# podmortem/log-parser

Hardware: AMD Instinct MI355X
Metric: log-lines/sec parsed+scored (whole node), 1k-pattern library (higher is better)
Workload: dtype fp64

## Files before the change

### csrc/bind.cpp

```cpp
#include <pybind11/numpy.h>
#include <pybind11/pybind11.h>
#include <pybind11/stl.h>

#include <atomic>
#include <chrono>
#include <condition_variable>
#include <cstring>
#include <deque>
#include <memory>
#include <mutex>
#include <thread>

#include "io/docs.h"
#include "io/json_in.h"
#include "io/loadgen.h"
#include "io/http_server.h"
#include "io/json_emit.h"
#include "kernels/lp_api.h"
#include "kernels/lp_host.h"
#include "regex/jregex.h"
#include "runtime/proc_shared.h"
#include "runtime/request.h"

namespace py = pybind11;
using namespace lp;

template <typename T>
static T* P(uint64_t v) { return reinterpret_cast<T*>(v); }

static PfTables pf_from(const py::tuple& t) {
  PfTables T;
  T.bloom = P<const uint32_t>(t[0].cast<uint64_t>());
  T.bloom_bits = t[1].cast<int>();
  T.ht_key = P<const uint64_t>(t[2].cast<uint64_t>());
  T.ht_val = P<const int32_t>(t[3].cast<uint64_t>());
  T.ht_cnt = P<const int32_t>(t[4].cast<uint64_t>());
  T.ht_mask = t[5].cast<uint32_t>();
  T.gram_lits = P<const int32_t>(t[6].cast<uint64_t>());
  T.lit_off = P<const int32_t>(t[7].cast<uint64_t>());
  T.lit_bytes = P<const uint8_t>(t[8].cast<uint64_t>());
  T.lit_reg_off = P<const int32_t>(t[9].cast<uint64_t>());
  T.lit_reg = P<const int32_t>(t[10].cast<uint64_t>());
  T.gmask = t[11].cast<int>();
  T.stride = t[12].cast<int>();
  T.teddy = P<const uint32_t>(t[13].cast<uint64_t>());
  T.tb_off = P<const int32_t>(t[14].cast<uint64_t>());
  T.tb_lits = P<const int32_t>(t[15].cast<uint64_t>());
  T.teddy_on = t[16].cast<int>();
  if (t.size() > 18) {
    T.gram_fp = P<const uint64_t>(t[17].cast<uint64_t>());
    T.tb_fp = P<const uint64_t>(t[18].cast<uint64_t>());
  }
  return T;
}

static DfaPool dfa_from(const py::tuple& t) {
  DfaPool D;
  D.meta = P<const int32_t>(t[0].cast<uint64_t>());
  D.bytemap = P<const uint8_t>(t[1].cast<uint64_t>());
  D.trans = P<const uint16_t>(t[2].cast<uint64_t>());
  D.acc = P<const uint8_t>(t[3].cast<uint64_t>());
  D.bpg = t.size() > 4 ? P<const uint64_t>(t[4].cast<uint64_t>()) : nullptr;
  D.bpg_widths = t.size() > 5 ? t[5].cast<uint32_t>() : 0u;
  D.bpg_words = t.size() > 6 ? t[6].cast<uint32_t>() : 0u;
  return D;
}

static GapTab gt_from(const py::tuple& t) {
  GapTab T;
  T.key = P<int64_t>(t[0].cast<uint64_t>());
  T.count = P<unsigned long long>(t[1].cast<uint64_t>());
  T.first = P<long long>(t[2].cast<uint64_t>());
  T.docs = P<int32_t>(t[3].cast<uint64_t>());
  T.last_doc = P<int32_t>(t[4].cast<uint64_t>());
  T.used = P<unsigned long long>(t[5].cast<uint64_t>());
  T.cap = t[6].cast<int64_t>();
  return T;
}

static GapRows gr_from(const py::tuple& t) {
  GapRows R;
  R.sig = P<int64_t>(t[0].cast<uint64_t>());
  R.count = P<int64_t>(t[1].cast<uint64_t>());
  R.first = P<int64_t>(t[2].cast<uint64_t>());
// ... 805 lines not shown
    return py::make_tuple(py::bytes(out.data(), k), intact);
  });

  m.def("line_index_tiles", &line_index_tiles);
  m.def("line_index_dev", [](uint64_t text, int64_t n, uint64_t ws, int64_t ntiles_cap, uint64_t starts, uint64_t lens,
                             int64_t cap, uint64_t info, bool trim, uint64_t blk, int64_t nblk, uint64_t s, bool counted) {
    line_index_dev(P<const uint8_t>(text), n, LineIndexWs{P<int64_t>(ws), ntiles_cap, size_t(1) << 20}, P<int64_t>(starts),
                   P<int32_t>(lens), cap, P<int64_t>(info), trim, P<int32_t>(blk), nblk, s, counted); },
        py::arg("text"), py::arg("n"), py::arg("ws"), py::arg("ntiles_cap"), py::arg("starts"), py::arg("lens"),
        py::arg("cap"), py::arg("info"), py::arg("trim"), py::arg("blk"), py::arg("nblk"), py::arg("s"),
        py::arg("counted") = false);
  m.def("prefilter_dev", [](uint64_t text, int64_t n, py::tuple pf, uint64_t ls, int64_t nl, uint64_t cand, int64_t cap,
                            uint64_t count, int grid, uint64_t s, py::object nlp) {
    NlOut o;
    const bool fused = !nlp.is_none();
    if (fused) {
      py::tuple t = nlp.cast<py::tuple>();
      o.nlm = P<uint64_t>(t[0].cast<uint64_t>());
      o.cnt = P<int32_t>(t[1].cast<uint64_t>());
      o.crf = P<int32_t>(t[2].cast<uint64_t>());
      o.ntiles = t[3].cast<int64_t>();
    }
    prefilter_dev(P<const uint8_t>(text), n, pf_from(pf), P<const int64_t>(ls), nl, P<int64_t>(cand), cap,
                  P<unsigned long long>(count), grid, s, fused ? &o : nullptr); },
        py::arg("text"), py::arg("n"), py::arg("pf"), py::arg("ls"), py::arg("nl"), py::arg("cand"), py::arg("cap"),
        py::arg("count"), py::arg("grid"), py::arg("s"), py::arg("nlp") = py::none());
  m.def("line_index_pass1", [](uint64_t ws, int64_t ntiles_cap, int64_t n, uint64_t s) {
    const NlOut o = line_index_pass1_views(LineIndexWs{P<int64_t>(ws), ntiles_cap, size_t(1) << 20}, n, s);
    return py::make_tuple(reinterpret_cast<uint64_t>(o.nlm), reinterpret_cast<uint64_t>(o.cnt),
                          reinterpret_cast<uint64_t>(o.crf), o.ntiles);
  });
  m.def("pf_verify_dev", [](uint64_t gh, int64_t n, uint64_t text, int64_t nb, py::tuple pf, uint64_t ls, int64_t nl,
                            uint64_t blk, uint64_t cand, int64_t cap, uint64_t count, uint64_t s, uint64_t dn,
                            int max_grid) {
    pf_verify_dev(P<const int64_t>(gh), n, P<const uint8_t>(text), nb, pf_from(pf), P<const int64_t>(ls), nl,
                  P<const int32_t>(blk), P<int64_t>(cand), cap, P<unsigned long long>(count), s,
                  P<const unsigned long long>(dn), max_grid); }, py::arg("gh"), py::arg("n"), py::arg("text"),
        py::arg("nb"), py::arg("pf"), py::arg("ls"), py::arg("nl"), py::arg("blk"), py::arg("cand"), py::arg("cap"),
        py::arg("count"), py::arg("s"), py::arg("dn") = 0, py::arg("max_grid") = 8192);
  m.def("append_keys", [](uint64_t dst, int64_t cap, uint64_t count, uint64_t src, int64_t n, uint64_t s) {
    append_keys_dev(P<int64_t>(dst), cap, P<unsigned long long>(count), P<const int64_t>(src), n, s); });
  m.def("take_host", [](uint64_t cand, uint64_t n1d, int64_t cap1, uint64_t ver, uint64_t n2d, int64_t cap2,
                        uint64_t text, uint64_t ls, uint64_t ll, py::tuple dfa, py::object out, uint64_t s) {
    HostSideOut O;
    if (!out.is_none()) {
      py::tuple t = out.cast<py::tuple>();
      O.keys = P<int64_t>(t[0].cast<uint64_t>()); O.starts = P<int64_t>(t[1].cast<uint64_t>());
      O.lens = P<int64_t>(t[2].cast<uint64_t>()); O.cap = t[3].cast<int64_t>();
      O.cnt = P<unsigned long long>(t[4].cast<uint64_t>()); O.done_blocks = P<unsigned int>(t[5].cast<uint64_t>());
      O.host_cnt = P<int64_t>(t[6].cast<uint64_t>()); O.host_seq = P<int64_t>(t[7].cast<uint64_t>());
      O.seq = t[8].cast<int64_t>();
    }
    take_host_dev(P<int64_t>(cand), P<const unsigned long long>(n1d), cap1, P<int64_t>(ver),
                  P<const unsigned long long>(n2d), cap2, P<const uint8_t>(text), P<const int64_t>(ls),
                  P<const int32_t>(ll), dfa_from(dfa), O, s); });
  m.def("wait_host", [](uint64_t ver, int64_t cap2, uint64_t n2d, py::tuple in, uint64_t s, double timeout_s) {
    HostSideIn I;
    I.keys = P<const int64_t>(in[0].cast<uint64_t>()); I.host_cnt = P<const int64_t>(in[1].cast<uint64_t>());
    I.host_seq = P<const int64_t>(in[2].cast<uint64_t>()); I.cap = in[3].cast<int64_t>(); I.seq = in[4].cast<int64_t>();
    I.err = P<int64_t>(in[5].cast<uint64_t>());
    I.timeout_ticks = (long long)(timeout_s * 1e8);
    wait_host_dev(P<int64_t>(ver), cap2, P<unsigned long long>(n2d), I, s); }, py::arg("ver"), py::arg("cap2"),
    py::arg("n2d"), py::arg("in"), py::arg("stream"), py::arg("timeout_s") = 2.0);
  m.def("host_alloc_coherent", [](int64_t bytes) {
    void* h = nullptr;
    if (hipHostMalloc(&h, (size_t)std::max<int64_t>(bytes, 8), hipHostMallocMapped | hipHostMallocCoherent) != hipSuccess)
      throw std::runtime_error("hipHostMalloc (coherent) failed");
    std::memset(h, 0, (size_t)std::max<int64_t>(bytes, 8));
    void* d = nullptr;
    if (hipHostGetDevicePointer(&d, h, 0) != hipSuccess) {
      (void)hipHostFree(h);
      throw std::runtime_error("hipHostGetDevicePointer failed");
// ... 697 lines not shown
```

### csrc/kernels/lp_api.h

```cpp
#pragma once
#include <stdint.h>

#include <vector>

#include "lp_core.h"

namespace lp {

void set_host_threads(int n);
void set_pf_verify_lanes(int n);
bool scan_defer_rare();
void set_scan_defer_rare(bool on);
void set_cand_verify_split(bool on);
bool summ_select();
void set_summ_select(bool on);
void set_small_profile(uint64_t dev_ptr);
struct NlOut {
  uint64_t* nlm = nullptr;
  int32_t* cnt = nullptr;
  int32_t* crf = nullptr;
  int64_t ntiles = 0;
};
void prefilter_dev(const uint8_t* text, int64_t nbytes, const PfTables& T, const int64_t* line_start, int64_t nlines,
                   int64_t* cand, int64_t cap, unsigned long long* count, int grid, uint64_t stream,
                   const NlOut* nl = nullptr);
void pf_verify_dev(const int64_t* ghits, int64_t n, const uint8_t* text, int64_t nbytes, const PfTables& T,
                   const int64_t* line_start, int64_t nlines, const int32_t* blk_line, int64_t* cand, int64_t cap,
                   unsigned long long* count, uint64_t stream, const unsigned long long* dn = nullptr,
                   int max_grid = 8192);
void bpg_cand_dev(int64_t* cand, int64_t cap, const unsigned long long* dcount, const uint8_t* text, const int64_t* ls,
                  const int32_t* ll, const DfaPool& P, uint64_t stream);
bool cand_verify_all_dev(int64_t* cand, int64_t cap, const unsigned long long* dcount, const uint8_t* text,
                         const int64_t* ls, const int32_t* ll, const DfaPool& P, uint64_t stream);
bool bpg_dedupe_dev(const uint64_t* keys, int64_t n, int lbits, const uint8_t* text, const int64_t* ls,
                    const int32_t* ll, const DfaPool& P, uint8_t* flag, uint64_t stream, uint32_t* wcnt = nullptr,
                    uint32_t* wlist = nullptr, int64_t* std_key = nullptr);
void bpg_scan_dev(const uint8_t* text, const int64_t* ls, const int32_t* ll, int64_t L, const int32_t* regs,
                  int nregs, const DfaPool& P, int64_t* out, int64_t cap, unsigned long long* count,
                  uint64_t stream);
struct HostSideOut {
  int64_t* keys = nullptr;
  int64_t* starts = nullptr;
  int64_t* lens = nullptr;
  int64_t cap = 0;
  unsigned long long* cnt = nullptr;
  unsigned int* done_blocks = nullptr;
  int64_t* host_cnt = nullptr;
  int64_t* host_seq = nullptr;
  int64_t seq = 0;
};
struct HostSideIn {
  const int64_t* keys = nullptr;
  const int64_t* host_cnt = nullptr;
  const int64_t* host_seq = nullptr;
  int64_t cap = 0;
  int64_t seq = 0;
  long long timeout_ticks = 200000000;
  int64_t* err = nullptr;
};
void take_host_dev(int64_t* cand, const unsigned long long* n1d, int64_t cap1, int64_t* ver,
                   const unsigned long long* n2d, int64_t cap2, const uint8_t* text, const int64_t* ls,
                   const int32_t* ll, const DfaPool& P, const HostSideOut& O, uint64_t stream);
// ... 334 lines not shown
```

### csrc/kernels/lp_core.h

```cpp
#pragma once
#include <hip/hip_runtime.h>
#include <stdint.h>

#define LP_HD __host__ __device__ __forceinline__

namespace lp {

template <typename T, int U = 8>
__device__ __forceinline__ void lds_fill(T* dst, const T* __restrict__ src, int n) {
  for (int b = threadIdx.x; b < n; b += U * (int)blockDim.x) {
    T v[U];
#pragma unroll
    for (int j = 0; j < U; ++j) {
      const int i = b + j * (int)blockDim.x;
      v[j] = src[i < n ? i : n - 1];
    }
#pragma unroll
    for (int j = 0; j < U; ++j) {
      const int i = b + j * (int)blockDim.x;
      if (i < n) dst[i] = v[j];
    }
  }
}

// ... 131 lines not shown
  if (ftl) {
    for (int k = 0; k < 4; ++k)
      if (st[k] >= 2 && (D[k].A[st[k]] & 2)) st[k] = 1;
    advance(s + ft, ftl);
  }
  uint32_t res = 0;
  for (int k = 0; k < 4; ++k)
    if (st[k] == 1 || (st[k] >= 2 && (D[k].A[st[k]] & 1))) res |= 1u << k;
  const uint8_t f = (res & 1u) ? 1 : ((res & 2u) ? 2 : 0);
  return (uint8_t)(f | (res & 12u));
#endif
}

struct PfTables {
  const uint32_t* bloom;
  int bloom_bits;
  const uint64_t* ht_key;
  const int32_t* ht_val;
  const int32_t* ht_cnt;
  uint32_t ht_mask;
  const int32_t* gram_lits;
  const int32_t* lit_off;
  const uint8_t* lit_bytes;
  const int32_t* lit_reg_off;
  const int32_t* lit_reg;
  int gmask;
  int stride;
  const uint32_t* teddy;
  const int32_t* tb_off;
  const int32_t* tb_lits;
  int teddy_on;
  const uint64_t* gram_fp = nullptr;
  const uint64_t* tb_fp = nullptr;
};

constexpr int LIT_OFF_SHIFT = 22;
LP_HD int pf_entry_lit(int32_t e) { return e & ((1 << LIT_OFF_SHIFT) - 1); }
LP_HD int pf_entry_off(int32_t e) { return (int)((uint32_t)e >> LIT_OFF_SHIFT); }

LP_HD uint32_t gram_mask(int g) { return g >= 4 ? 0xFFFFFFFFu : ((1u << (8 * g)) - 1u); }
LP_HD uint32_t bloom_hash(uint32_t key, int g) { return (key ^ (uint32_t)g * 0x9E3779B9u) * 0x85EBCA6Bu; }
LP_HD uint32_t bloom_word(uint32_t key, int g, int bits) {
  return bloom_hash(key, g) >> (32 - (bits - 5));
}
LP_HD uint32_t bloom_bits_of(uint32_t p) {
  const uint32_t q = p ^ (p >> 15);
  return (1u << (q & 31)) | (1u << ((q >> 5) & 31)) | (1u << ((q >> 10) & 31));
}
LP_HD uint32_t bloom_bits2(uint32_t key, int g) { return bloom_bits_of(bloom_hash(key, g)); }
LP_HD bool bloom_test(const uint32_t* bl, uint32_t key, int g, int bits) {
  const uint32_t p = bloom_hash(key, g);
  const uint32_t m = bloom_bits_of(p);
  return (bl[p >> (32 - (bits - 5))] & m) == m;
}
LP_HD uint32_t ht_hash(uint32_t key, int g) {
  uint32_t h = key * 0x9E3779B1u ^ ((uint32_t)g * 0x7FEB352Du);
  h ^= h >> 15;
  h *= 0x2C1B3C6Du;
  h ^= h >> 12;
  return h;
}
LP_HD int lower_byte(int c) { return (c >= 'A' && c <= 'Z') ? c + 32 : c; }
LP_HD uint32_t lower4(uint32_t x) {
  uint32_t hi = 0x80808080u;
  uint32_t ge_A = ((x | hi) - 0x41414141u) & hi;
  uint32_t ge_Z1 = ((x | hi) - 0x5B5B5B5Bu) & hi;
  uint32_t up = ge_A & ~ge_Z1 & ~x & hi;
// ... 33 lines not shown
#if defined(__HIP__)
__device__ __forceinline__ void load16u(const uint8_t* p, uint32_t out[4]) {
  const int sh = (int)((uintptr_t)p & 15);
  const uint4* b = reinterpret_cast<const uint4*>(p - sh);
  const uint4 x = b[0], y = b[1];
  uint32_t a0 = x.x, a1 = x.y, a2 = x.z, a3 = x.w, a4 = y.x, a5 = y.y, a6 = y.z, a7 = y.w;
  const int q = sh >> 2, r = sh & 3;
  if (q & 2) { a0 = a2; a1 = a3; a2 = a4; a3 = a5; a4 = a6; a5 = a7; }
  if (q & 1) { a0 = a1; a1 = a2; a2 = a3; a3 = a4; a4 = a5; }
  out[0] = __builtin_amdgcn_alignbyte(a1, a0, r);
  out[1] = __builtin_amdgcn_alignbyte(a2, a1, r);
  out[2] = __builtin_amdgcn_alignbyte(a3, a2, r);
  out[3] = __builtin_amdgcn_alignbyte(a4, a3, r);
}
__device__ __forceinline__ bool lit_match16(const uint8_t* t, const uint8_t* lit, int len) {
  for (int q = 0; q < len; q += 16) {
    uint32_t a[4], b[4];
    load16u(t + q, a);
    load16u(lit + q, b);
    const int rem = len - q;
    uint32_t diff = 0;
#pragma unroll
    for (int i = 0; i < 4; ++i) {
      const int k = rem - 4 * i;
      const uint32_t m = k >= 4 ? 0xFFFFFFFFu : (k <= 0 ? 0u : ((1u << (8 * k)) - 1u));
      diff |= (lower4(a[i]) ^ b[i]) & m;
    }
    if (diff) return false;
  }
  return true;
}
#endif

LP_HD void pf_bucket(const PfTables& T, uint32_t gram, int g, int& s, int& c) {
  const uint64_t key = (uint64_t)gram | ((uint64_t)g << 32);
  uint32_t h = ht_hash(gram, g) & T.ht_mask;
  s = 0;
  c = 0;
  for (;;) {
    const uint64_t kk = T.ht_key[h];
    if (kk == ~0ull) return;
    if (kk == key) break;
    h = (h + 1) & T.ht_mask;
  }
  s = T.ht_val[h];
  c = T.ht_cnt[h];
}

LP_HD bool pf_lit_at(const PfTables& T, const uint8_t* text, int64_t nbytes, int64_t p, int32_t e) {
  const int lit = pf_entry_lit(e);
  const int lo = T.lit_off[lit], len = T.lit_off[lit + 1] - lo;
  const int64_t st = p - pf_entry_off(e);
  if (st < 0 || st + len > nbytes) return false;
#if defined(__HIP_DEVICE_COMPILE__)
  return lit_match16(text + st, T.lit_bytes + lo, len);
#else
  for (int q = 0; q < len; ++q)
    if (lower_byte(text[st + q]) != T.lit_bytes[lo + q]) return false;
  return true;
#endif
}

template <typename AppendFn>
LP_HD void pf_probe(const PfTables& T, const uint8_t* text, int64_t nbytes, int64_t p, uint32_t gram, int g,
                    const int64_t* line_start, int64_t nlines, const int32_t* blk_line, AppendFn&& append) {
  int s, c;
  pf_bucket(T, gram, g, s, c);
  int64_t line = -1;
  for (int j = 0; j < c; ++j) {
    const int32_t e = T.gram_lits[s + j];
    if (!pf_lit_at(T, text, nbytes, p, e)) continue;
    const int lit = pf_entry_lit(e);
    if (line < 0) line = locate_line(line_start, nlines, blk_line, p);
    if (line < 0) line = 0;
    for (int r = T.lit_reg_off[lit]; r < T.lit_reg_off[lit + 1]; ++r)
      append(((int64_t)T.lit_reg[r] << 32) | line);
  }
}

LP_HD uint32_t teddy_mask(const PfTables& T, const uint8_t* text, int64_t nbytes, int64_t p) {
  const int b0 = lower_byte(text[p]);
  const int b1 = p + 1 < nbytes ? lower_byte(text[p + 1]) : 0;
  const int b2 = p + 2 < nbytes ? lower_byte(text[p + 2]) : 0;
  return T.teddy[4 * b0] & T.teddy[4 * b1 + 1] & T.teddy[4 * b2 + 2];
}

template <typename AppendFn>
LP_HD void teddy_probe(const PfTables& T, const uint8_t* text, int64_t nbytes, int64_t p, uint32_t m,
                       const int64_t* line_start, int64_t nlines, const int32_t* blk_line, AppendFn&& append) {
  int64_t line = -1;
  while (m) {
    const int b = __builtin_ctz(m);
    m &= m - 1;
    for (int j = T.tb_off[b]; j < T.tb_off[b + 1]; ++j) {
      const int32_t e = T.tb_lits[j];
      if (!pf_lit_at(T, text, nbytes, p, e)) continue;
      const int lit = pf_entry_lit(e);
      if (line < 0) line = locate_line(line_start, nlines, blk_line, p);
      if (line < 0) line = 0;
      for (int r = T.lit_reg_off[lit]; r < T.lit_reg_off[lit + 1]; ++r)
        append(((int64_t)T.lit_reg[r] << 32) | line);
    }
  }
// ... 198 lines not shown
```

### csrc/kernels/lp_kernels.hip

```cpp
#include <hip/hip_runtime.h>

#include <algorithm>
#include <cstdlib>
#include <cstdio>
#include <cstring>
#include <stdexcept>
#include <string>
#include <thread>
#include <vector>

#include "lp_api.h"
#include "lp_core.h"
#include "lp_host.h"

namespace lp {

#define LP_CHECK(x)                                                                           \
  do {                                                                                        \
    hipError_t e_ = (x);                                                                      \
    if (e_ != hipSuccess) throw std::runtime_error(std::string("HIP error: ") + hipGetErrorString(e_) + " at " #x); \
  } while (0)

static inline hipStream_t as_stream(uint64_t s) { return reinterpret_cast<hipStream_t>(s); }

// ... 215 lines not shown
  if (dn) {
    const int64_t d = (int64_t)*dn;
    n = d < n ? d : n;
  }
  const LdsAppender app{buf, &cnt, cand, cap, count};
  constexpr int HITS_PER_BLOCK = 256 / PV_LANES;
  const int sub = threadIdx.x / PV_LANES, lane = threadIdx.x % PV_LANES;
  const int64_t stride = (int64_t)gridDim.x * HITS_PER_BLOCK;
  for (int64_t base = (int64_t)blockIdx.x * HITS_PER_BLOCK; base < n; base += stride) {
    const int64_t i = base + sub;
    if (i < n) {
      const int64_t h = ghits[i];
      const int64_t p = h >> 2;
      const bool td = (h & 3) == 3;
      const int G = td ? 3 : 2 + (int)(h & 3);
      uint32_t a[4];
      if (p >= 4) {
        load16u(text + p - 4, a);
      } else {
        for (int k = 0; k < 4; ++k) {
          uint32_t v = 0;
          for (int b = 3; b >= 0; --b) {
            const int64_t x = p - 4 + 4 * k + b;
            v = (v << 8) | (x >= 0 ? (uint32_t)text[x] : 0u);
          }
          a[k] = v;
        }
      }
#pragma unroll
      for (int k = 0; k < 4; ++k) a[k] = lower4(a[k]);
      const uint64_t t8 = (uint64_t)a[0] |
                          ((uint64_t)(G == 4 ? a[2] : __builtin_amdgcn_alignbyte(a[2], a[1], G)) << 32);
      int64_t line = -1;
      auto walk = [&](const int32_t* ents, const uint64_t* fps, int j0, int j1) {
        for (int j = j0 + lane; j < j1; j += PV_LANES) {
          const uint4 f = *reinterpret_cast<const uint4*>(fps + 2 * j);
          const uint64_t fp = (uint64_t)f.x | ((uint64_t)f.y << 32), fm = (uint64_t)f.z | ((uint64_t)f.w << 32);
          if ((t8 ^ fp) & fm) continue;
          const int32_t e = ents[j];
          if (!pf_lit_at(T, text, nbytes, p, e)) continue;
          const int lit = pf_entry_lit(e);
          if (line < 0) line = locate_line(line_start, nlines, blk_line, p);
          if (line < 0) line = 0;
          for (int r = T.lit_reg_off[lit]; r < T.lit_reg_off[lit + 1]; ++r) app(((int64_t)T.lit_reg[r] << 32) | line);
        }
      };
      if (td) {
        const uint32_t b1 = p + 1 < nbytes ? (a[1] >> 8) & 0xFF : 0u, b2 = p + 2 < nbytes ? (a[1] >> 16) & 0xFF : 0u;
        uint32_t m = T.teddy[4 * (a[1] & 0xFF)] & T.teddy[4 * b1 + 1] & T.teddy[4 * b2 + 2];
        while (m) {
          const int b = __ffs(m) - 1;
          m &= m - 1;
          walk(T.tb_lits, T.tb_fp, T.tb_off[b], T.tb_off[b + 1]);
        }
      } else {
        int s0, c;
        pf_bucket(T, a[1] & gram_mask(G), G, s0, c);
        walk(T.gram_lits, T.gram_fp, s0, s0 + c);
      }
    }
    __syncthreads();
    const int c = *reinterpret_cast<volatile int*>(&cnt);
    if (c >= PF_BUF / 2) pf_flush(buf, &cnt, &gbase, c, cand, cap, count);
  }
  __syncthreads();
  const int c = *reinterpret_cast<volatile int*>(&cnt);
  if (c > 0) pf_flush(buf, &cnt, &gbase, c, cand, cap, count);
}

__global__ __launch_bounds__(256) void k_scan(const uint8_t* __restrict__ text,
                                              const int64_t* __restrict__ line_start,
                                              const int32_t* __restrict__ line_len, int64_t nlines,
                                              const int32_t* __restrict__ regs, int nregs, DfaPool P,
                                              int64_t* out, int64_t cap, unsigned long long* count) {
  const int64_t line = (int64_t)blockIdx.x * blockDim.x + threadIdx.x;
  if (line >= nlines) return;
  const uint8_t* s = text + line_start[line];
  const int n = line_len[line];
  const Appender app{out, cap, count};
  for (int j = 0; j < nregs; ++j) {
    const int r = regs[j];
    if (dfa_run(P, r, s, n)) app(((int64_t)r << 32) | line);
  }
}

constexpr int kScoreEv = 64;
__global__ __launch_bounds__(4 * kScoreEv) void k_score(const int32_t* __restrict__ ev_line,
                                                        const int32_t* __restrict__ ev_pat,
                                                        const int32_t* __restrict__ ev_seg, FreqIn F,
                                                        int64_t n, ScoreTables T, ScoreParams S,
                                                        double* __restrict__ out, double* __restrict__ factors,
// ... 70 lines not shown
    case 4: LP_PF(4, 1); break;
    case 8: LP_PF(8, 1); break;
    case 12: LP_PF(12, 1); break;
    case 16: LP_PF(16, 1); break;
    case 20: LP_PF(20, 1); break;
    case 24: LP_PF(24, 1); break;
    default: LP_PF(28, 1); break;
  }
#undef LP_PF
}

void prefilter_dev(const uint8_t* text, int64_t nbytes, const PfTables& T, const int64_t* line_start, int64_t nlines,
                   int64_t* cand, int64_t cap, unsigned long long* count, int grid, uint64_t stream, const NlOut* nl) {
  if (nbytes <= 0 || ((T.gmask & 28) == 0 && !T.teddy_on)) {
    if (nl) throw std::runtime_error("prefilter_dev: the fused line-index pass needs a prefilter");
    return;
  }
  const int64_t units = (nbytes + 15) / 16;
  const bool big = nbytes >= (int64_t(32) << 20);
  const int threads = T.teddy_on ? pf_threads<true>() : pf_threads<false>();
  const int g = (int)std::min<int64_t>(grid, num_blocks(units, threads * (big ? 4 : 1)));
  if (T.teddy_on)
    dispatch_pf<true>(g, big, as_stream(stream), text, nbytes, T, line_start, nlines, cand, cap, count, nl);
  else
    dispatch_pf<false>(g, big, as_stream(stream), text, nbytes, T, line_start, nlines, cand, cap, count, nl);
  LP_CHECK(hipGetLastError());
}

static int g_pv_lanes_bulk = 4;
void set_pf_verify_lanes(int n) { g_pv_lanes_bulk = (n == 1 || n == 2 || n == 4 || n == 16) ? n : 4; }

void pf_verify_dev(const int64_t* ghits, int64_t n, const uint8_t* text, int64_t nbytes, const PfTables& T,
                   const int64_t* line_start, int64_t nlines, const int32_t* blk_line, int64_t* cand, int64_t cap,
                   unsigned long long* count, uint64_t stream, const unsigned long long* dn, int max_grid) {
  if (n <= 0) return;
  const int lanes = nbytes >= (int64_t(64) << 20) ? g_pv_lanes_bulk : 16;
  const int64_t need = (n + 256 / lanes - 1) / (256 / lanes);
  const int g = dn ? (int)std::min<int64_t>(need, std::max(1, max_grid)) : (int)std::max<int64_t>(1, need);
#define LP_PV(L)                                                                                                  \
  hipLaunchKernelGGL(k_pf_verify<L>, dim3(g), dim3(256), 0, as_stream(stream), ghits, n, dn, text, nbytes, T, \
                     line_start, nlines, blk_line, cand, cap, count)
  switch (lanes) {
    case 1: LP_PV(1); break;
    case 2: LP_PV(2); break;
    case 4: LP_PV(4); break;
    default: LP_PV(16); break;
  }
#undef LP_PV
  LP_CHECK(hipGetLastError());
}

__global__ __launch_bounds__(256) void k_append_keys(int64_t* __restrict__ dst, int64_t cap,
                                                     unsigned long long* __restrict__ count,
                                                     const int64_t* __restrict__ src, int64_t n) {
  __shared__ unsigned long long base;
  const int64_t b0 = (int64_t)blockIdx.x * blockDim.x;
  const int64_t nb = min((int64_t)blockDim.x, n - b0);
  if (threadIdx.x == 0) base = atomicAdd(count, (unsigned long long)nb);
  __syncthreads();
  const int64_t i = b0 + threadIdx.x;
  if (i < n && (int64_t)(base + threadIdx.x) < cap) dst[base + threadIdx.x] = src[i];
}

void append_keys_dev(int64_t* dst, int64_t cap, unsigned long long* count, const int64_t* src, int64_t n,
                     uint64_t stream) {
  if (n <= 0) return;
  hipLaunchKernelGGL(k_append_keys, dim3((unsigned)((n + 255) / 256)), dim3(256), 0,
                     reinterpret_cast<hipStream_t>(stream), dst, cap, count, src, n);
  hipError_t e = hipGetLastError();
// ... 151 lines not shown
```

### log_parser_amd/models/compiled.py

```python
from __future__ import annotations

import logging
from dataclasses import dataclass, field
from typing import Dict, List, Optional, Sequence, Tuple

import numpy as np
import torch

from ..golden import CONTEXT_REGEXES, SEVERITY_MULTIPLIERS, java_blank, severity_key
from ..native import N
from ..utils.config import ScoringParams
from .nfa import build_group, fits_group, pack_groups
from .schema import Pattern, PatternSet, pattern_to_json

log = logging.getLogger("log_parser_amd.compiled")

KIND_DFA, KIND_NFA, KIND_FALLBACK, KIND_INVALID = 0, 1, 2, 3
RELAX = "(?#relax)"
BLOOM_BITS = 18


def _minimize_literals(lits: List[bytes]) -> List[bytes]:
    s = sorted(set(lits), key=len)
    out: List[bytes] = []
    for x in s:
        if not any(y in x for y in out):
            out.append(x)
    return out


_FREQ = {**{c: f * 0.55 for c, f in zip(b"etaoinshrdlcumwfgypbvkjxqz",
                                         (12.7, 9.1, 8.2, 7.5, 7.0, 6.7, 6.3, 6.1, 6.0, 4.3, 4.0, 2.8, 2.8, 2.4,
                                          2.4, 2.2, 2.0, 2.0, 1.9, 1.5, 1.0, 0.8, 0.15, 0.15, 0.1, 0.07))},
         **{c: 3.0 for c in b"0123456789"}, ord(" "): 14.0, ord("."): 1.5, ord(":"): 1.5, ord("-"): 1.2,
         ord("="): 0.6, ord("/"): 0.6, ord("_"): 0.5, ord("["): 0.4, ord("]"): 0.4, ord(","): 0.5,
         ord("("): 0.3, ord(")"): 0.3, ord("\t"): 0.5}


PF_STRIDE_MAX = 4
PF_TEDDY = True
TEDDY_MIN, TEDDY_MAX = 3, 6
TEDDY_BUCKETS = 32
TEDDY_MAX_LITS = 2048
MIN_LITERAL = 3

LIT_OFF_SHIFT = 22
MAX_GRAM_OFF = (1 << (31 - LIT_OFF_SHIFT)) - 1


def _window_cost(w: bytes) -> float:
    import math
    return sum(math.log2(_FREQ.get(c, 0.05) / 100.0) for c in w)


def _choose_grams(lits: List[bytes], stride: int = 1) -> List[List[Tuple[int, int, int]]]:
    import math
    used: Dict[Tuple[int, int], int] = {}
    out = []
    for lit in lits:
        g = min(4, len(lit))
        best = None
        for i in range(min(len(lit) - g - stride + 1, MAX_GRAM_OFF - stride + 1) + 1):
            alpha = 0.5 if stride == 1 else 0.75
            cost = math.log2(sum(
                2.0 ** (_window_cost(lit[i + d:i + d + g])
                        + alpha * math.log2(1 + used.get((int.from_bytes(lit[i + d:i + d + g], "little"), g), 0)))
                for d in range(stride)))
            if best is None or (cost, i) < best:
                best = (cost, i)
        ents = []
        for d in range(stride):
            off = best[1] + d
            key = int.from_bytes(lit[off:off + g], "little")
            used[(key, g)] = used.get((key, g), 0) + 1
            ents.append((key, g, off))
        out.append(ents)
    return out


def _fingerprint(lit: bytes, off: int, g: int) -> Tuple[int, int]:
    fp = mask = 0
    for k in range(4):
        i = off - 4 + k
        if 0 <= i < len(lit):
            fp |= lit[i] << (8 * k)
            mask |= 0xFF << (8 * k)
    for k in range(4):
        i = off + g + k
        if i < len(lit):
            fp |= lit[i] << (32 + 8 * k)
            mask |= 0xFF << (32 + 8 * k)
    return fp, mask


def _fingerprints(entries: Sequence[int], lits: List[bytes], gs: Sequence[int]) -> np.ndarray:
    out = np.zeros(2 * max(len(entries), 1), np.uint64)
    for j, e in enumerate(entries):
        lit = lits[e & ((1 << LIT_OFF_SHIFT) - 1)]
        fp, mask = _fingerprint(lit, e >> LIT_OFF_SHIFT, gs[j])
        out[2 * j], out[2 * j + 1] = np.uint64(fp), np.uint64(mask)
    return out


def _teddy_tables(lits: List[bytes], ids: List[int]):
    tab = np.zeros((256, 4), np.uint32)
    if not lits:
        return tab, np.zeros(TEDDY_BUCKETS + 1, np.int32), np.zeros(1, np.int32)
    win = []
    for lit, i in zip(lits, ids):
        o = min(range(len(lit) - 2), key=lambda k: (_window_cost(lit[k:k + 3]), k))
        win.append((lit[o:o + 3], o, i))
    win.sort()
    B = min(TEDDY_BUCKETS, len(win))
    members: List[List[int]] = [[] for _ in range(TEDDY_BUCKETS)]
    for r, (w, o, i) in enumerate(win):
        b = r * B // len(win)
        for j in range(3):
            tab[w[j], j] |= np.uint32(1 << b)
        members[b].append(i | (o << LIT_OFF_SHIFT))
    off = np.zeros(TEDDY_BUCKETS + 1, np.int32)
    for b in range(TEDDY_BUCKETS):
        off[b + 1] = off[b] + len(members[b])
    ent = np.array([e for m in members for e in m] or [0], np.int32)
    return tab, off, ent


def _u32(x):
    return x & 0xFFFFFFFF


def bloom_hash(key, g):
    return _u32((key ^ _u32(g * 0x9E3779B9)) * 0x85EBCA6B)


# ... 453 lines not shown
        for i, rr in enumerate(lit_regs):
            lit_reg_off[i + 1] = lit_reg_off[i] + len(rr)
        lit_reg = np.array([r for rr in lit_regs for r in rr] or [0], np.int32)
        short = []
        if PF_TEDDY:
            short = [i for i, l in enumerate(lits) if TEDDY_MIN <= len(l) <= TEDDY_MAX and 0 not in l]
            short = short[:TEDDY_MAX_LITS]
        sset = set(short)
        long_ids = [i for i in range(len(lits)) if i not in sset]
        teddy, tb_off, tb_lits = _teddy_tables([lits[i] for i in short], short)
        grams: Dict[Tuple[int, int], List[int]] = {}
        gmask = 0
        stride = 1
        if long_ids and len(lits) < (1 << LIT_OFF_SHIFT):
            shortest = min(len(lits[i]) for i in long_ids)
            for s_ in (4, 2):
                if PF_STRIDE_MAX >= s_ and shortest >= s_ + 3:
                    stride = s_
                    break
        for i, ents in zip(long_ids, _choose_grams([lits[i] for i in long_ids], stride)):
            for key, g, off in ents:
                grams.setdefault((key, g), []).append(i | (off << LIT_OFF_SHIFT))
                gmask |= 1 << g
        bits = BLOOM_BITS
        bloom = np.zeros((1 << bits) // 32, np.uint32)
        for key, g in grams:
            bloom[bloom_word(key, g, bits)] |= np.uint32(bloom_bits2(key, g))
        H = 16
        while H < 2 * max(1, len(grams)):
            H *= 2
        ht_key = np.full(H, np.uint64(0xFFFFFFFFFFFFFFFF), np.uint64)
        ht_val = np.zeros(H, np.int32)
        ht_cnt = np.zeros(H, np.int32)
        gram_lits: List[int] = []
        gram_g: List[int] = []
        for (key, g), ids in grams.items():
            h = ht_hash(key, g) & (H - 1)
            while ht_key[h] != np.uint64(0xFFFFFFFFFFFFFFFF):
                h = (h + 1) & (H - 1)
            ht_key[h] = np.uint64(key | (g << 32))
            ht_val[h] = len(gram_lits)
            ht_cnt[h] = len(ids)
            gram_lits.extend(ids)
            gram_g.extend([g] * len(ids))
        gram_fp = _fingerprints(gram_lits, lits, gram_g)
        ntb = int(tb_off[-1])
        tb_fp = _fingerprints([int(x) for x in tb_lits[:ntb]], lits, [3] * ntb)
        self.pf = dict(gram_g=np.array(gram_g or [4], np.int32), bloom=bloom, bits=bits, ht_key=ht_key, ht_val=ht_val, ht_cnt=ht_cnt, ht_mask=H - 1,
                       gram_fp=gram_fp, tb_fp=tb_fp,
                       gram_lits=np.array(gram_lits or [0], np.int32), lit_off=lit_off, lit_bytes=lit_bytes,
                       lit_reg_off=lit_reg_off, lit_reg=lit_reg, gmask=gmask, stride=stride,
                       teddy=teddy, tb_off=tb_off, tb_lits=tb_lits, teddy_lits=len(short))

    def device_tables(self, device: torch.device) -> dict:
        key = str(device)
        t = self._device_cache.get(key)
        if t is not None:
            return t

        def T(a):
            return torch.from_numpy(np.ascontiguousarray(a)).to(device)

        t = {}
        pf = self.pf
        t["pf_arrays"] = [T(pf["bloom"]), T(pf["ht_key"].view(np.int64)), T(pf["ht_val"]), T(pf["ht_cnt"]),
                          T(pf["gram_lits"]), T(pf["lit_off"]), T(pf["lit_bytes"]), T(pf["lit_reg_off"]),
                          T(pf["lit_reg"]), T(pf["teddy"]), T(pf["tb_off"]), T(pf["tb_lits"]),
                          T(pf["gram_fp"].view(np.int64)), T(pf["tb_fp"].view(np.int64))]
        a = t["pf_arrays"]
        t["pf"] = (a[0].data_ptr(), pf["bits"], a[1].data_ptr(), a[2].data_ptr(), a[3].data_ptr(), pf["ht_mask"],
                   a[4].data_ptr(), a[5].data_ptr(), a[6].data_ptr(), a[7].data_ptr(), a[8].data_ptr(), pf["gmask"],
                   pf["stride"], a[9].data_ptr(), a[10].data_ptr(), a[11].data_ptr(), 1 if pf["teddy_lits"] else 0,
                   a[12].data_ptr(), a[13].data_ptr())
        t["dfa_arrays"] = [T(self.dfa_meta), T(self.dfa_bytemap), T(self.dfa_trans.view(np.int16)), T(self.dfa_acc),
                           T(self.bpg_pool.view(np.int64))]
        d = t["dfa_arrays"]
        t["dfa"] = (d[0].data_ptr(), d[1].data_ptr(), d[2].data_ptr(), d[3].data_ptr(), d[4].data_ptr(),
                    self.bpg_widths, int(self.bpg_pool.size))
        t["scan_regs"] = T(np.array(self.scan_regs_single, np.int32))
        t["scan_blobs"] = [T(p["blob"]) for p in self.scan_passes]
        t["scan_passes"] = [(b.data_ptr(), p["lds_words"], p["ngroups"], p["row_base"], p["stride"], p["thr"],
                             p["init_row"], p["init_state"], p["ncol"], p["gt_off"], p["fin_off"], p["bm_off"],
                             p["rid_off"], p["am_off"], p["gm_off"]) for b, p in zip(t["scan_blobs"], self.scan_passes)]
        t["conf"], t["sev"] = T(self.conf), T(self.sev)
        t["sev_index"] = T(self.sev_index)
        t["ctx_before"], t["ctx_after"] = T(self.ctx_before), T(self.ctx_after)
        t["sec_off"], t["sec_reg"], t["sec_w"], t["sec_weight"] = T(self.sec_off), T(self.sec_reg), T(self.sec_w), T(self.sec_weight)
        t["seq_off"], t["seq_bonus"], t["seq_ev_off"], t["seq_ev_reg"] = T(self.seq_off), T(self.seq_bonus), T(self.seq_ev_off), T(self.seq_ev_reg)
        slot_seq = np.zeros(max(self.n_seq_events, 1), np.int32)
        for q in range(len(self.seq_off) and (self.seq_ev_off.size - 1)):
            slot_seq[self.seq_ev_off[q]:self.seq_ev_off[q + 1]] = q
        t["slot_seq"] = T(slot_seq)
        t["prim_off"], t["prim_pats"] = T(self.prim_off), T(self.prim_pats)
        t["prim_cnt"] = T(np.diff(self.prim_off))
        t["freq_key"] = T(self.freq_key)
        t["is_primary"] = T(np.diff(self.prim_off) > 0)
        t["host_dev"] = bool(self.host_dev)
        t["nfa_tables"] = T(self.nfa_tables.view(np.int64))
        t["nfa_ctx_list"] = T(np.array(self.nfa_ctx_groups, np.int32))
        t["nfa_scan_lists"] = {k: T(np.array([g for g in self.nfa_scan_groups if self.nfa_group_ncls[g] == k], np.int32))
                               for k in (1, 2, 3)}
        self._device_cache[key] = t
        return t

    @property
    def ctx_dfa_extent(self) -> Tuple[int, int]:
# ... 27 lines not shown
```

### log_parser_amd/ops/kernels.py

```python
from __future__ import annotations

from typing import Optional, Tuple

import torch

from ..native import N

TEXT_PAD = 64
NL_TILE = 16384


def _s(t: torch.Tensor) -> int:
    return torch.cuda.current_stream(t.device).cuda_stream if t.is_cuda else 0


def _p(t: Optional[torch.Tensor]) -> int:
    return 0 if t is None else t.data_ptr()


def padded_len(nbytes: int) -> int:
    return ((max(nbytes, 1) + NL_TILE - 1) // NL_TILE) * NL_TILE + TEXT_PAD


def newline_positions(text: torch.Tensor, nbytes: int) -> torch.Tensor:
# ... 107 lines not shown

def split_chunk_lines(text: torch.Tensor, nbytes: int) -> Tuple[torch.Tensor, torch.Tensor]:
    dev = text.device
    if text.is_cuda and nbytes > 0:
        starts, lens, n_nl, last, _, blk = _line_index_dev(text, nbytes, trim=False)
        L = n_nl + 1 - (1 if n_nl and last == nbytes - 1 else 0)
        return _with_blk(starts[:L], blk, nbytes), lens[:L]
    nl = newline_positions(text.cpu(), nbytes).to(dev)
    zero = torch.zeros(1, dtype=torch.int64, device=dev)
    starts = torch.cat([zero, nl + 1])
    ends = torch.cat([nl, torch.full((1,), nbytes, dtype=torch.int64, device=dev)])
    if nl.numel():
        prev = text[(nl - 1).clamp(min=0)]
        cr = (nl > starts[:-1]) & (prev == 13)
        ends[:-1] -= cr.to(torch.int64)
    L = starts.numel()
    if nl.numel() and int(nl[-1].item()) == nbytes - 1:
        L -= 1
    return starts[:L].contiguous(), (ends - starts)[:L].to(torch.int32).contiguous()




def line_block_index(line_start: torch.Tensor, nbytes: int) -> torch.Tensor:
    cached = getattr(line_start, "_lp_blk", None)
    if cached is not None and cached[1] == nbytes:
        return cached[0]
    nblk = (max(nbytes, 1) >> LINE_BLK_SHIFT) + 2
    blk = torch.empty(nblk, dtype=torch.int32, device=line_start.device)
    N.blk_index(line_start.data_ptr(), line_start.numel(), nblk, blk.data_ptr(), _s(line_start), line_start.is_cuda)
    return blk


def prefilter(text, nbytes, pf_tuple, line_start, cap: int, grid: int = 2048) -> torch.Tensor:
    nlines = line_start.numel()
    if text.is_cuda:
        dev = text.device
        gcap = cap
        blk = line_block_index(line_start, nbytes)
        while True:
            gh = torch.empty(max(gcap, 1), dtype=torch.int64, device=dev)
            cand = torch.empty(max(cap, 1), dtype=torch.int64, device=dev)
            cnt = torch.zeros(2, dtype=torch.int64, device=dev)
            N.prefilter_dev(text.data_ptr(), nbytes, pf_tuple, line_start.data_ptr(), nlines, gh.data_ptr(), gcap,
                            cnt.data_ptr(), grid, _s(text))
            N.pf_verify_dev(gh.data_ptr(), gcap, text.data_ptr(), nbytes, pf_tuple, line_start.data_ptr(), nlines,
                            blk.data_ptr(), cand.data_ptr(), cap, cnt.data_ptr() + 8, _s(text), cnt.data_ptr(),
                            max(16, min(8192, nbytes >> 13)))
            c = cnt.cpu()
            g, k = int(c[0]), int(c[1])
            if g <= gcap and k <= cap:
                return cand[:k]
            gcap, cap = max(gcap, g), max(cap, k)
    while True:
        cand = torch.empty(max(cap, 1), dtype=torch.int64)
        c = N.prefilter_host(text.data_ptr(), nbytes, pf_tuple, line_start.data_ptr(), nlines, cand.data_ptr(), cap)
        if c <= cap:
            return cand[:c]
        cap = c


def scan(text, line_start, line_len, regs: torch.Tensor, dfa_tuple, cap: int) -> torch.Tensor:
    nlines = line_start.numel()
    if regs.numel() == 0 or nlines == 0:
        return torch.empty(0, dtype=torch.int64, device=text.device)
    if text.is_cuda:
        while True:
            out = torch.empty(max(cap, 1), dtype=torch.int64, device=text.device)
            cnt = torch.zeros(1, dtype=torch.int64, device=text.device)
            N.scan_dev(text.data_ptr(), line_start.data_ptr(), line_len.data_ptr(), nlines, regs.data_ptr(),
                       regs.numel(), dfa_tuple, out.data_ptr(), cap, cnt.data_ptr(), _s(text))
            c = int(cnt.item())
            if c <= cap:
                return out[:c]
            cap = c
    while True:
        out = torch.empty(max(cap, 1), dtype=torch.int64)
        c = N.scan_host(text.data_ptr(), line_start.data_ptr(), line_len.data_ptr(), nlines, regs.data_ptr(),
                        regs.numel(), dfa_tuple, out.data_ptr(), cap)
        if c <= cap:
            return out[:c]
# ... 818 lines not shown
```

Measured before the change: 516.8 million.

## Split large prefilter gram buckets by a context byte to shrink verify walks

At compile time, gram hash buckets with more than eight literals are partitioned on the context byte (of the eight surrounding bytes) that best separates their fingerprints. Each split bucket gets a 256-entry offset table, and literals that do not constrain that byte stay in an always-checked open prefix. At probe time, both the device verify kernel and the host path read the text byte at that position and walk only the open prefix plus the matching sub-range, instead of every literal in the bucket. This adds one table load and some index arithmetic per probe, plus extra context-byte reads on the host path. A lanes override argument is also plumbed through to pf_verify_dev.

Result: no change. 521.3 million, median of 3 (+0.9%).

```diff
diff --git a/csrc/bind.cpp b/csrc/bind.cpp
--- a/csrc/bind.cpp
+++ b/csrc/bind.cpp
@@ -50,6 +50,10 @@
   if (t.size() > 18) {
     T.gram_fp = P<const uint64_t>(t[17].cast<uint64_t>());
     T.tb_fp = P<const uint64_t>(t[18].cast<uint64_t>());
+  }
+  if (t.size() > 20) {
+    T.ht_sub = P<const int32_t>(t[19].cast<uint64_t>());
+    T.sub_tab = P<const uint16_t>(t[20].cast<uint64_t>());
   }
   return T;
 }
@@ -921,12 +925,12 @@
   });
   m.def("pf_verify_dev", [](uint64_t gh, int64_t n, uint64_t text, int64_t nb, py::tuple pf, uint64_t ls, int64_t nl,
                             uint64_t blk, uint64_t cand, int64_t cap, uint64_t count, uint64_t s, uint64_t dn,
-                            int max_grid) {
+                            int max_grid, int lanes) {
     pf_verify_dev(P<const int64_t>(gh), n, P<const uint8_t>(text), nb, pf_from(pf), P<const int64_t>(ls), nl,
                   P<const int32_t>(blk), P<int64_t>(cand), cap, P<unsigned long long>(count), s,
-                  P<const unsigned long long>(dn), max_grid); }, py::arg("gh"), py::arg("n"), py::arg("text"),
+                  P<const unsigned long long>(dn), max_grid, lanes); }, py::arg("gh"), py::arg("n"), py::arg("text"),
         py::arg("nb"), py::arg("pf"), py::arg("ls"), py::arg("nl"), py::arg("blk"), py::arg("cand"), py::arg("cap"),
-        py::arg("count"), py::arg("s"), py::arg("dn") = 0, py::arg("max_grid") = 8192);
+        py::arg("count"), py::arg("s"), py::arg("dn") = 0, py::arg("max_grid") = 8192, py::arg("lanes") = 0);
   m.def("append_keys", [](uint64_t dst, int64_t cap, uint64_t count, uint64_t src, int64_t n, uint64_t s) {
     append_keys_dev(P<int64_t>(dst), cap, P<unsigned long long>(count), P<const int64_t>(src), n, s); });
   m.def("take_host", [](uint64_t cand, uint64_t n1d, int64_t cap1, uint64_t ver, uint64_t n2d, int64_t cap2,
diff --git a/csrc/kernels/lp_api.h b/csrc/kernels/lp_api.h
--- a/csrc/kernels/lp_api.h
+++ b/csrc/kernels/lp_api.h
@@ -27,7 +27,7 @@
 void pf_verify_dev(const int64_t* ghits, int64_t n, const uint8_t* text, int64_t nbytes, const PfTables& T,
                    const int64_t* line_start, int64_t nlines, const int32_t* blk_line, int64_t* cand, int64_t cap,
                    unsigned long long* count, uint64_t stream, const unsigned long long* dn = nullptr,
-                   int max_grid = 8192);
+                   int max_grid = 8192, int lanes = 0);
 void bpg_cand_dev(int64_t* cand, int64_t cap, const unsigned long long* dcount, const uint8_t* text, const int64_t* ls,
                   const int32_t* ll, const DfaPool& P, uint64_t stream);
 bool cand_verify_all_dev(int64_t* cand, int64_t cap, const unsigned long long* dcount, const uint8_t* text,
diff --git a/csrc/kernels/lp_core.h b/csrc/kernels/lp_core.h
--- a/csrc/kernels/lp_core.h
+++ b/csrc/kernels/lp_core.h
@@ -187,7 +187,10 @@
   int teddy_on;
   const uint64_t* gram_fp = nullptr;
   const uint64_t* tb_fp = nullptr;
-};
+  const int32_t* ht_sub = nullptr;
+  const uint16_t* sub_tab = nullptr;
+};
+constexpr int PF_SUB_STRIDE = 258;
 
 constexpr int LIT_OFF_SHIFT = 22;
 LP_HD int pf_entry_lit(int32_t e) { return e & ((1 << LIT_OFF_SHIFT) - 1); }
@@ -287,19 +290,42 @@
 }
 #endif
 
-LP_HD void pf_bucket(const PfTables& T, uint32_t gram, int g, int& s, int& c) {
+LP_HD void pf_bucket(const PfTables& T, uint32_t gram, int g, int& s, int& c, int& slot) {
   const uint64_t key = (uint64_t)gram | ((uint64_t)g << 32);
   uint32_t h = ht_hash(gram, g) & T.ht_mask;
   s = 0;
   c = 0;
   for (;;) {
     const uint64_t kk = T.ht_key[h];
+    slot = (int)h;
     if (kk == ~0ull) return;
     if (kk == key) break;
     h = (h + 1) & T.ht_mask;
   }
   s = T.ht_val[h];
   c = T.ht_cnt[h];
+}
+
+LP_HD void pf_sub_range(const PfTables& T, int slot, int s, int c, uint64_t t8, int& n_open, int& j0, int& j1) {
+  const int sv = T.ht_sub ? T.ht_sub[slot] : -1;
+  n_open = c;
+  j0 = j1 = s + c;
+  if (sv < 0) return;
+  const uint16_t* sub = T.sub_tab + (int64_t)(sv >> 3) * PF_SUB_STRIDE;
+  const int b = (int)(t8 >> (8 * (sv & 7))) & 0xFF;
+  n_open = sub[0];
+  j0 = s + n_open + sub[1 + b];
+  j1 = s + n_open + sub[2 + b];
+}
+
+LP_HD uint64_t pf_context(const uint8_t* text, int64_t nbytes, int64_t p, int g) {
+  uint64_t t8 = 0;
+  for (int k = 0; k < 4; ++k) {
+    const int64_t x = p - 4 + k, y = p + g + k;
+    if (x >= 0) t8 |= (uint64_t)lower_byte(text[x]) << (8 * k);
+    if (y < nbytes) t8 |= (uint64_t)lower_byte(text[y]) << (32 + 8 * k);
+  }
+  return t8;
 }
 
 LP_HD bool pf_lit_at(const PfTables& T, const uint8_t* text, int64_t nbytes, int64_t p, int32_t e) {
@@ -319,11 +345,14 @@
 template <typename AppendFn>
 LP_HD void pf_probe(const PfTables& T, const uint8_t* text, int64_t nbytes, int64_t p, uint32_t gram, int g,
                     const int64_t* line_start, int64_t nlines, const int32_t* blk_line, AppendFn&& append) {
-  int s, c;
-  pf_bucket(T, gram, g, s, c);
+  int s, c, slot, n_open, j0, j1;
+  pf_bucket(T, gram, g, s, c, slot);
+  if (c == 0) return;
+  pf_sub_range(T, slot, s, c, pf_context(text, nbytes, p, g), n_open, j0, j1);
   int64_t line = -1;
-  for (int j = 0; j < c; ++j) {
-    const int32_t e = T.gram_lits[s + j];
+  const int n = n_open + (j1 - j0);
+  for (int k = 0; k < n; ++k) {
+    const int32_t e = T.gram_lits[k < n_open ? s + k : j0 + (k - n_open)];
     if (!pf_lit_at(T, text, nbytes, p, e)) continue;
     const int lit = pf_entry_lit(e);
     if (line < 0) line = locate_line(line_start, nlines, blk_line, p);
diff --git a/csrc/kernels/lp_kernels.hip b/csrc/kernels/lp_kernels.hip
--- a/csrc/kernels/lp_kernels.hip
+++ b/csrc/kernels/lp_kernels.hip
@@ -271,8 +271,10 @@
       const uint64_t t8 = (uint64_t)a[0] |
                           ((uint64_t)(G == 4 ? a[2] : __builtin_amdgcn_alignbyte(a[2], a[1], G)) << 32);
       int64_t line = -1;
-      auto walk = [&](const int32_t* ents, const uint64_t* fps, int j0, int j1) {
-        for (int j = j0 + lane; j < j1; j += PV_LANES) {
+      auto walk = [&](const int32_t* ents, const uint64_t* fps, int s, int n0, int j0, int j1) {
+        const int nw = n0 + (j1 - j0);
+        for (int k = lane; k < nw; k += PV_LANES) {
+          const int j = k < n0 ? s + k : j0 + (k - n0);
           const uint4 f = *reinterpret_cast<const uint4*>(fps + 2 * j);
           const uint64_t fp = (uint64_t)f.x | ((uint64_t)f.y << 32), fm = (uint64_t)f.z | ((uint64_t)f.w << 32);
           if ((t8 ^ fp) & fm) continue;
@@ -290,12 +292,14 @@
         while (m) {
           const int b = __ffs(m) - 1;
           m &= m - 1;
-          walk(T.tb_lits, T.tb_fp, T.tb_off[b], T.tb_off[b + 1]);
+          const int t0 = T.tb_off[b], t1 = T.tb_off[b + 1];
+          walk(T.tb_lits, T.tb_fp, t0, t1 - t0, t1, t1);
         }
       } else {
-        int s0, c;
-        pf_bucket(T, a[1] & gram_mask(G), G, s0, c);
-        walk(T.gram_lits, T.gram_fp, s0, s0 + c);
+        int s0, c, slot, n_open, j0, j1;
+        pf_bucket(T, a[1] & gram_mask(G), G, s0, c, slot);
+        pf_sub_range(T, slot, s0, c, t8, n_open, j0, j1);
+        walk(T.gram_lits, T.gram_fp, s0, n_open, j0, j1);
       }
     }
     __syncthreads();
@@ -432,9 +436,11 @@
 
 void pf_verify_dev(const int64_t* ghits, int64_t n, const uint8_t* text, int64_t nbytes, const PfTables& T,
                    const int64_t* line_start, int64_t nlines, const int32_t* blk_line, int64_t* cand, int64_t cap,
-                   unsigned long long* count, uint64_t stream, const unsigned long long* dn, int max_grid) {
+                   unsigned long long* count, uint64_t stream, const unsigned long long* dn, int max_grid,
+                   int pin_lanes) {
   if (n <= 0) return;
-  const int lanes = nbytes >= (int64_t(64) << 20) ? g_pv_lanes_bulk : 16;
+  if (pin_lanes != 0 && pin_lanes != 4 && pin_lanes != 16) throw std::runtime_error("pf_verify_dev: lanes is 0, 4 or 16");
+  const int lanes = pin_lanes ? pin_lanes : nbytes >= (int64_t(64) << 20) ? g_pv_lanes_bulk : 16;
   const int64_t need = (n + 256 / lanes - 1) / (256 / lanes);
   const int g = dn ? (int)std::min<int64_t>(need, std::max(1, max_grid)) : (int)std::max<int64_t>(1, need);
 #define LP_PV(L)                                                                                                  \
diff --git a/log_parser_amd/models/compiled.py b/log_parser_amd/models/compiled.py
--- a/log_parser_amd/models/compiled.py
+++ b/log_parser_amd/models/compiled.py
@@ -38,6 +38,8 @@
 
 
 PF_STRIDE_MAX = 4
+PF_SPLIT_MIN = 8
+PF_SUB_STRIDE = 258
 PF_TEDDY = True
 TEDDY_MIN, TEDDY_MAX = 3, 6
 TEDDY_BUCKETS = 32
@@ -100,6 +102,24 @@
         fp, mask = _fingerprint(lit, e >> LIT_OFF_SHIFT, gs[j])
         out[2 * j], out[2 * j + 1] = np.uint64(fp), np.uint64(mask)
     return out
+
+
+def _split_bucket(ids: Sequence[int], lits: List[bytes], g: int) -> Tuple[List[int], int, np.ndarray]:
+    fm = [_fingerprint(lits[e & ((1 << LIT_OFF_SHIFT) - 1)], e >> LIT_OFF_SHIFT, g) for e in ids]
+    best = None
+    for q in range(8):
+        n_open = sum(1 for _, m in fm if not (m >> (8 * q)) & 0xFF)
+        nb = np.bincount([(f >> (8 * q)) & 0xFF for f, m in fm if (m >> (8 * q)) & 0xFF], minlength=256)
+        cost = n_open * len(ids) + int((nb.astype(np.int64) ** 2).sum())
+        if best is None or cost < best[0]:
+            best = (cost, q)
+    q = best[1]
+    opened = sorted(e for e, (_, m) in zip(ids, fm) if not (m >> (8 * q)) & 0xFF)
+    rest = sorted(((f >> (8 * q)) & 0xFF, e) for e, (f, m) in zip(ids, fm) if (m >> (8 * q)) & 0xFF)
+    sub = np.zeros(PF_SUB_STRIDE, np.uint16)
+    sub[0] = len(opened)
+    sub[2:] = np.cumsum(np.bincount([b for b, _ in rest], minlength=256))
+    return opened + [e for _, e in rest], q, sub
 
 
 def _teddy_tables(lits: List[bytes], ids: List[int]):
@@ -619,12 +639,18 @@
         ht_key = np.full(H, np.uint64(0xFFFFFFFFFFFFFFFF), np.uint64)
         ht_val = np.zeros(H, np.int32)
         ht_cnt = np.zeros(H, np.int32)
+        ht_sub = np.full(H, -1, np.int32)
+        subs: List[np.ndarray] = []
         gram_lits: List[int] = []
         gram_g: List[int] = []
         for (key, g), ids in grams.items():
             h = ht_hash(key, g) & (H - 1)
             while ht_key[h] != np.uint64(0xFFFFFFFFFFFFFFFF):
                 h = (h + 1) & (H - 1)
+            if PF_SPLIT_MIN < len(ids) <= 0xFFFF:
+                ids, q, sub = _split_bucket(ids, lits, g)
+                ht_sub[h] = (len(subs) << 3) | q
+                subs.append(sub)
             ht_key[h] = np.uint64(key | (g << 32))
             ht_val[h] = len(gram_lits)
             ht_cnt[h] = len(ids)
@@ -634,7 +660,8 @@
         ntb = int(tb_off[-1])
         tb_fp = _fingerprints([int(x) for x in tb_lits[:ntb]], lits, [3] * ntb)
         self.pf = dict(gram_g=np.array(gram_g or [4], np.int32), bloom=bloom, bits=bits, ht_key=ht_key, ht_val=ht_val, ht_cnt=ht_cnt, ht_mask=H - 1,
-                       gram_fp=gram_fp, tb_fp=tb_fp,
+                       gram_fp=gram_fp, tb_fp=tb_fp, ht_sub=ht_sub,
+                       sub_tab=np.concatenate(subs) if subs else np.zeros(PF_SUB_STRIDE, np.uint16),
                        gram_lits=np.array(gram_lits or [0], np.int32), lit_off=lit_off, lit_bytes=lit_bytes,
                        lit_reg_off=lit_reg_off, lit_reg=lit_reg, gmask=gmask, stride=stride,
                        teddy=teddy, tb_off=tb_off, tb_lits=tb_lits, teddy_lits=len(short))
@@ -653,12 +680,13 @@
         t["pf_arrays"] = [T(pf["bloom"]), T(pf["ht_key"].view(np.int64)), T(pf["ht_val"]), T(pf["ht_cnt"]),
                           T(pf["gram_lits"]), T(pf["lit_off"]), T(pf["lit_bytes"]), T(pf["lit_reg_off"]),
                           T(pf["lit_reg"]), T(pf["teddy"]), T(pf["tb_off"]), T(pf["tb_lits"]),
-                          T(pf["gram_fp"].view(np.int64)), T(pf["tb_fp"].view(np.int64))]
+                          T(pf["gram_fp"].view(np.int64)), T(pf["tb_fp"].view(np.int64)),
+                          T(pf["ht_sub"]), T(pf["sub_tab"].view(np.int16))]
         a = t["pf_arrays"]
         t["pf"] = (a[0].data_ptr(), pf["bits"], a[1].data_ptr(), a[2].data_ptr(), a[3].data_ptr(), pf["ht_mask"],
                    a[4].data_ptr(), a[5].data_ptr(), a[6].data_ptr(), a[7].data_ptr(), a[8].data_ptr(), pf["gmask"],
                    pf["stride"], a[9].data_ptr(), a[10].data_ptr(), a[11].data_ptr(), 1 if pf["teddy_lits"] else 0,
-                   a[12].data_ptr(), a[13].data_ptr())
+                   a[12].data_ptr(), a[13].data_ptr(), a[14].data_ptr(), a[15].data_ptr())
         t["dfa_arrays"] = [T(self.dfa_meta), T(self.dfa_bytemap), T(self.dfa_trans.view(np.int16)), T(self.dfa_acc),
                            T(self.bpg_pool.view(np.int64))]
         d = t["dfa_arrays"]
diff --git a/log_parser_amd/ops/kernels.py b/log_parser_amd/ops/kernels.py
--- a/log_parser_amd/ops/kernels.py
+++ b/log_parser_amd/ops/kernels.py
@@ -163,7 +163,7 @@
     return blk
 
 
-def prefilter(text, nbytes, pf_tuple, line_start, cap: int, grid: int = 2048) -> torch.Tensor:
+def prefilter(text, nbytes, pf_tuple, line_start, cap: int, grid: int = 2048, lanes: int = 0) -> torch.Tensor:
     nlines = line_start.numel()
     if text.is_cuda:
         dev = text.device
@@ -177,7 +177,7 @@
                             cnt.data_ptr(), grid, _s(text))
             N.pf_verify_dev(gh.data_ptr(), gcap, text.data_ptr(), nbytes, pf_tuple, line_start.data_ptr(), nlines,
                             blk.data_ptr(), cand.data_ptr(), cap, cnt.data_ptr() + 8, _s(text), cnt.data_ptr(),
-                            max(16, min(8192, nbytes >> 13)))
+                            max(16, min(8192, nbytes >> 13)), lanes)
             c = cnt.cpu()
             g, k = int(c[0]), int(c[1])
             if g <= gcap and k <= cap:
```
